# barbararoessle/e2e_multi_view_matching

Measured on AMD Instinct MI355X. Metric: image-pairs/sec @1024 kpts + pose AUC@5/10/20deg vs reference, higher is better.
Workload: dtype f16x2 (fp32 operands carried as 2 fp16 planes hi + 2^-11 lo', 22 significant bits, 3 fp16-MFMA products, fp32 accumulate; same 1e-4 / bit-exact-index parity bar); 1 GPU; configs[1]: tuple_size=2 (1 pair per tuple), 1024 keypoints, 256-dim f32 descriptors, GNN 9x1 = 18 layers, 100 Sinkhorn iters, batch 32 tuples/GPU = 32 pairs/GPU, w8pt pose per pair; pairs_per_gpu=32, global_pairs=32, weights=random init (timed), identity-like for the AUC leg, parallelism=tuple-sharded x1

## Files before the change

e2e_multi_view_matching_amd/csrc/attention_p2w.hip:

```cpp
#include <algorithm>
#include <type_traits>

#include "attention_p2.h"

namespace e2emv {

typedef __attribute__((ext_vector_type(16))) float aw_f32x16;

constexpr int AW_QT = 256;
constexpr int AW_TILEB = 64 * 256;
constexpr int AW_REGB = 2 * AW_TILEB;
constexpr int AW_ELS = 3 * AW_REGB;
constexpr int AW_QIMG = AW_ELS + 2048;
constexpr int AW_LDS = AW_QIMG + 3 * AW_TILEB;
constexpr int AW_PART_F = 68;
constexpr float AW_SINV = 1.f / P2_QS, AW_PLOG = 7.f, AW_LIMIT = 60000.f;

__device__ __forceinline__ void aw_wait_q_k0(p2_f16x8 (&q)[2][2][4]) {
    asm volatile("s_waitcnt vmcnt(0) lgkmcnt(0)\n\ts_barrier"
                 : "+a"(q[0][0][0]), "+a"(q[0][0][1]), "+a"(q[0][0][2]), "+a"(q[0][0][3]), "+a"(q[0][1][0]), "+a"(q[0][1][1]), "+a"(q[0][1][2]), "+a"(q[0][1][3]),
                   "+a"(q[1][0][0]), "+a"(q[1][0][1]), "+a"(q[1][0][2]), "+a"(q[1][0][3]), "+a"(q[1][1][0]), "+a"(q[1][1][1]), "+a"(q[1][1][2]), "+a"(q[1][1][3])
                 :: "memory");
}

template <int I, int N, class F>
__device__ __forceinline__ void aw_for(F&& f) {
    if constexpr (I < N) {
        f(std::integral_constant<int, I>{});
        aw_for<I + 1, N>(f);
    }
}

__device__ __forceinline__ unsigned aw_cvt_pk(float v0, float v1) {
    const p2_f32x2 vv = {v0, v1};
    return __builtin_bit_cast(unsigned, __builtin_convertvector(vv, p2_f16x2));
}
__device__ __forceinline__ float aw_fma(float a, float b, float c) {
    float d;
    asm volatile("v_fma_f32 %0, %1, %2, %3" : "=v"(d) : "v"(a), "v"(b), "v"(c));
    return d;
}
__device__ __forceinline__ float aw_exp2(float a) {
    float d;
    asm volatile("v_exp_f32 %0, %1" : "=v"(d) : "v"(a));
    return d;
}
__device__ __forceinline__ void aw_acc(float& sum, float a) { asm volatile("v_add_f32 %0, %0, %1" : "+v"(sum) : "v"(a)); }
__device__ __forceinline__ unsigned aw_cvt_pk_v(float v0, float v1) {
    unsigned d;
    asm volatile("v_cvt_pk_f16_f32 %0, %1, %2" : "=v"(d) : "v"(v0), "v"(v1));
    return d;
}
__device__ __forceinline__ unsigned aw_mixlo(unsigned hi, float v0) {
    unsigned lo;
    asm volatile("v_fma_mixlo_f16 %0, %1, -1.0, %2 op_sel_hi:[1,0,0]" : "=v"(lo) : "v"(hi), "v"(v0));
    return lo;
}
__device__ __forceinline__ unsigned aw_mixhi(unsigned lo, unsigned hi, float v1) {
    asm volatile("v_fma_mixhi_f16 %0, %1, -1.0, %2 op_sel:[1,0,0] op_sel_hi:[1,0,0]" : "+v"(lo) : "v"(hi), "v"(v1));
    return lo;
}
__device__ __forceinline__ unsigned aw_lo(unsigned hi, float v0, float v1) {
    unsigned lo;
    asm("v_fma_mixlo_f16 %0, %1, -1.0, %2 op_sel_hi:[1,0,0]\n\tv_fma_mixhi_f16 %0, %1, -1.0, %3 op_sel:[1,0,0] op_sel_hi:[1,0,0]"
        : "=&v"(lo) : "v"(hi), "v"(v0), "v"(v1));
    return lo;
}

__device__ __forceinline__ void aw_mfma_s(aw_f32x16& c, p2_f16x8 a, p2_f16x8 b) {
    asm volatile("v_mfma_f32_32x32x16_f16 %0, %1, %2, %0" : "+v"(c) : "v"(a), "a"(b));
}
__device__ __forceinline__ void aw_mfma_s0(aw_f32x16& c, p2_f16x8 a, p2_f16x8 b) {
    asm volatile("v_mfma_f32_32x32x16_f16 %0, %1, %2, 0" : "=&v"(c) : "v"(a), "a"(b));
}
__device__ __forceinline__ void aw_mfma_sa(aw_f32x16& c, p2_f16x8 a, p2_f16x8 b) {
    asm volatile("v_mfma_f32_32x32x16_f16 %0, %1, %2, %0" : "+v"(c) : "a"(a), "a"(b));
}
__device__ __forceinline__ void aw_mfma_sa0(aw_f32x16& c, p2_f16x8 a, p2_f16x8 b) {
    asm volatile("v_mfma_f32_32x32x16_f16 %0, %1, %2, 0" : "=&v"(c) : "a"(a), "a"(b));
}
__device__ __forceinline__ void aw_mfma_oa(aw_f32x16& c, p2_f16x8 a, p2_u32x4 b) {
    asm volatile("v_mfma_f32_32x32x16_f16 %0, %1, %2, %0" : "+a"(c) : "a"(a), "v"(b));
}
template <int IMM>
__device__ __forceinline__ void aw_read_frag(p2_f16x8& d, unsigned addr) {
    static_assert(IMM >= 0 && IMM < 65536, "ds_read offset: 16 bits");
    asm volatile("ds_read_b128 %0, %1 offset:%2" : "=a"(d) : "v"(addr), "n"(IMM));
}
template <int N>
__device__ __forceinline__ void aw_wait_frag(p2_f16x8 (&f)[4]) {
    asm volatile("s_waitcnt lgkmcnt(%4)" : "+a"(f[0]), "+a"(f[1]), "+a"(f[2]), "+a"(f[3]) : "n"(N));
}
template <bool HAS_E, bool MULTI = true, bool PART = false>
__global__ __launch_bounds__(256, 1) void attention_p2w_kernel(AttnP2Params p) {
    extern __shared__ __attribute__((aligned(16))) char smem_aw[];

    int lin = blockIdx.x, ks = 0;
    constexpr bool part = PART;
    if constexpr (PART) {
        const int h = blockIdx.x, tpx = (8 * p.gper * p.nq - p.n_full) >> 3;
        ks = (h >> 3) / tpx;
        lin = p.n_full + 8 * ((h >> 3) % tpx) + (h & 7);
    }
    const int xcd = lin & 7, idx = lin >> 3;
    const int g = xcd * p.gper + idx / p.nq;
    if (g >= p.groups) return;
    const int qt = idx % p.nq;
    const int img = g / p.H, head = g % p.H;
    const int b = img / p.T, t = img % p.T;
    if (qt * AW_QT >= p.nv[t]) return;

    const int tid = threadIdx.x, lane = tid & 63;
    const int wave = __builtin_amdgcn_readfirstlane(tid >> 6);
    const int l31 = lane & 31, lh = lane >> 5;
    const unsigned row_b = 8u * (unsigned)p.D;

    int q_row[2];
    bool q_ok[2];
    p2_f16x8 Qf[2][2][4];
#pragma unroll
    for (int a = 0; a < 2; ++a) {
        q_row[a] = qt * AW_QT + wave * 64 + a * 32 + l31;
        q_ok[a] = q_row[a] < p.n_rows;
    }
    const int q_blk = __builtin_amdgcn_readfirstlane(((int64_t)img * p.n_rows + min(qt * AW_QT + wave * 64, p.n_rows - 1)) >> 6);
    const int e_q_v = HAS_E ? p.EQK[q_blk * 8 + head] : 0;
    const unsigned q_img = wave == 0 ? 2u * AW_REGB : (unsigned)(AW_QIMG + (wave - 1) * AW_TILEB);
    {
        const __amdgpu_buffer_rsrc_t rsQ = __builtin_amdgcn_make_buffer_rsrc(const_cast<uint16_t*>(p.qk), 0, (int)p.qk_bytes, 0x00020000);
        const unsigned so = (unsigned)(img * p.n_rows) * row_b;
        asm volatile("" ::: "memory");
#pragma unroll
        for (int i = 0; i < 16; ++i) {
            const int rl = 4 * i + (lane >> 4);
            const int row = min(qt * AW_QT + wave * 64 + rl, p.n_rows - 1);
            const unsigned c = (unsigned)((lane & 15) ^ (rl & 15));
            p2_glds16(rsQ, smem_aw + q_img + i * 1024, (unsigned)row * row_b + (unsigned)head * 256u + c * 16u, so);
        }
        asm volatile("" ::: "memory");
    }
    const int e_q = __builtin_amdgcn_readfirstlane(e_q_v);

    const int n_src = p.cross ? p.T - 1 : 1;
    auto src_t = [&](int si) __attribute__((always_inline)) { return !p.cross ? t : (si < t ? si : si + 1); };
    int n_tiles = 0;
    for (int si = 0; si < n_src; ++si) n_tiles += (p.nv[src_t(si)] + 63) / 64;
    int t0 = 0;
    if constexpr (PART) {
        t0 = ks * n_tiles / p.n_split;
        n_tiles = (ks + 1) * n_tiles / p.n_split - t0;
        if (n_tiles <= 0) return;
    }
    struct Cur { int si, kt, nv; unsigned kb, vb; int eb; };
    auto cur_src = [&](Cur& c) __attribute__((always_inline)) {
        const int im = b * p.T + src_t(c.si);
        c.kt = 0;
        c.nv = p.nv[src_t(c.si)];
        c.kb = (unsigned)(im * p.n_rows) * row_b;
        c.vb = (unsigned)((im * p.H + head) * 64) * (unsigned)p.n_rows * 4u;
        c.eb = (im * p.n_rows) >> 6;
    };
    auto cur_next = [&](Cur& c) __attribute__((always_inline)) {
        ++c.kt;
        if constexpr (MULTI) {
            if (c.kt * 64 >= c.nv && c.si + 1 < n_src) { ++c.si; cur_src(c); }
        }
    };
    auto cur_init = [&]() __attribute__((always_inline)) {
        Cur c;
        c.si = 0;
        cur_src(c);
        if constexpr (PART)
            for (int i = 0; i < t0; ++i) cur_next(c);
        return c;
    };

    const __amdgpu_buffer_rsrc_t rsK = __builtin_amdgcn_make_buffer_rsrc(const_cast<uint16_t*>(p.qk), 0, (int)p.qk_bytes, 0x00020000);
    const __amdgpu_buffer_rsrc_t rsV = __builtin_amdgcn_make_buffer_rsrc(const_cast<uint16_t*>(p.vt), 0, (int)p.vt_bytes, 0x00020000);
    unsigned k_vo[4], v_vo[4];
#pragma unroll
    for (int i = 0; i < 4; ++i) {
        const int row = 4 * (wave * 4 + i) + (lane >> 4);
        const unsigned c = (unsigned)((lane & 15) ^ (row & 15));
        k_vo[i] = (unsigned)row * row_b + 4u * (unsigned)p.D + (unsigned)head * 256u + c * 16u;
        v_vo[i] = (unsigned)row * (unsigned)p.n_rows * 4u + c * 16u;
    }
    auto k_so = [&](const Cur& c) __attribute__((always_inline)) { return c.kb + (unsigned)c.kt * 64u * row_b; };
    auto v_so = [&](const Cur& c) __attribute__((always_inline)) { return c.vb + (unsigned)c.kt * 256u; };
    auto k_piece = [&](int region, int i, unsigned so) __attribute__((always_inline)) { p2_glds16(rsK, smem_aw + region * AW_REGB + AW_TILEB + (wave * 4 + i) * 1024, k_vo[i], so); };
    auto v_piece = [&](int region, int i, unsigned so) __attribute__((always_inline)) { p2_glds16(rsV, smem_aw + region * AW_REGB + (wave * 4 + i) * 1024, v_vo[i], so); };
    int* const els = reinterpret_cast<int*>(smem_aw + AW_ELS);
    int ek_mine = 0, ev_mine = 0;
    if (HAS_E && tid < n_tiles) {
        int si = 0, kt = PART ? tid + t0 : tid;
        if constexpr (MULTI) {
            for (; si + 1 < n_src; ++si) {
                const int nt = (p.nv[src_t(si)] + 63) / 64;
                if (kt < nt) break;
                kt -= nt;
            }
        }
        const int blk = (((b * p.T + src_t(si)) * p.n_rows) >> 6) + kt;
        ek_mine = p.EQK[blk * 8 + 4 + head];
        if (p.EVt) ev_mine = p.EVt[blk * 4 + head];
    }
    typedef __attribute__((address_space(3))) const p2_u32x2* lds_pair_t;
    const unsigned els0 = (unsigned)(uintptr_t)(__attribute__((address_space(3))) char*)smem_aw + (unsigned)AW_ELS;
    auto read_e = [&](int tl) __attribute__((always_inline)) {
        return *reinterpret_cast<lds_pair_t>((uintptr_t)(els0 + 8u * (unsigned)min(tl, n_tiles - 1)));
    };

    const int kz = l31 & 15;
    const unsigned lds0 = (unsigned)(uintptr_t)(__attribute__((address_space(3))) char*)smem_aw;
    unsigned R[4][2];
#pragma unroll
    for (int s = 0; s < 4; ++s)
#pragma unroll
        for (int pl = 0; pl < 2; ++pl)
            R[s][pl] = lds0 + (unsigned)(l31 * 256 + ((((s >> 1) * 8 + pl * 4 + 2 * (s & 1) + lh) ^ kz) << 4));
    typedef __attribute__((address_space(3))) const p2_f16x8* lds_frag_t;
    auto frag = [&](int s, int pl, int imm) __attribute__((always_inline)) { return *reinterpret_cast<lds_frag_t>((uintptr_t)(R[s][pl] + (unsigned)imm)); };

    constexpr int PA[3] = {1, 0, 0};
    constexpr int PB[3] = {0, 1, 0};

    aw_f32x16 O[2][2], S[2][2];
    p2_u32x4 Pf[2][2][4];
#pragma unroll
    for (int a = 0; a < 2; ++a)
#pragma unroll
        for (int d = 0; d < 2; ++d)
#pragma unroll
            for (int r = 0; r < 16; ++r) O[a][d][r] = 0.f;
    float m_run[2] = {-1e30f, -1e30f}, l_run[2] = {0.f, 0.f};
    int e_o = 0;
    bool o_started = false;
    unsigned n_slow = 0;

    auto sm_slow = [&](auto BB, float sinv, int valid) __attribute__((always_inline)) {
        constexpr int B = decltype(BB)::value;
        asm volatile("s_nop 15" : "+v"(S[B][0]), "+v"(S[B][1]), "+a"(O[B][0]), "+a"(O[B][1]));
        if (valid < 64) {
#pragma unroll
            for (int kb = 0; kb < 2; ++kb)
#pragma unroll
                for (int r = 0; r < 16; ++r)
                    if (kb * 32 + (r & 3) + 8 * (r >> 2) + 4 * lh >= valid) S[B][kb][r] = -INFINITY;
        }
        float mx = S[B][0][0];
#pragma unroll
        for (int kb = 0; kb < 2; ++kb)
#pragma unroll
            for (int r = 0; r < 16; ++r) mx = fmaxf(mx, S[B][kb][r]);
        {
            float x = mx, y = mx;
            asm volatile("s_nop 1\n\tv_permlane32_swap_b32 %0, %1\n\ts_nop 1" : "+v"(x), "+v"(y));
            mx = fmaxf(x, y);
        }
        mx *= sinv;
        const float m_new = fmaxf(m_run[B], mx);
        const float alpha = __builtin_amdgcn_exp2f(m_run[B] - m_new);
#pragma unroll
        for (int r = 0; r < 16; ++r) { O[B][0][r] *= alpha; O[B][1][r] *= alpha; }
        const float e0 = AW_PLOG - m_new;
        float ps = 0.f;
#pragma unroll
        for (int k = 0; k < 16; ++k) {
            const int kb = k >> 3, r = 2 * (k & 7), u = 2 * kb + ((k & 7) >> 2), e = k & 3;
            const float p0 = __builtin_amdgcn_exp2f(__builtin_fmaf(S[B][kb][r], sinv, e0));
            const float p1 = __builtin_amdgcn_exp2f(__builtin_fmaf(S[B][kb][r + 1], sinv, e0));
            ps += p0 + p1;
            const P2Pair pr = p2_split_plain(p0, p1);
            Pf[B][0][u][e] = pr.hi; Pf[B][1][u][e] = pr.lo;
        }
        l_run[B] = l_run[B] * alpha + ps;
        m_run[B] = m_new;
        asm volatile("s_nop 4" : "+a"(O[B][0]), "+a"(O[B][1]));
    };

    Cur cK = cur_init(), cV = cur_init(), cS = cur_init();
    int nK = 0, nV = 0;
    auto adv_k = [&]() __attribute__((always_inline)) { if (++nK < n_tiles) cur_next(cK); };
    auto adv_v = [&]() __attribute__((always_inline)) { if (++nV < n_tiles) cur_next(cV); };
    {
        const unsigned so = k_so(cK);
#pragma unroll
        for (int i = 0; i < 4; ++i) k_piece(2, i, so);
        adv_k();
    }
    unsigned so_v01[2], so_k12[2];
#pragma unroll
    for (int r = 0; r < 2; ++r) {
        so_v01[r] = v_so(cV);
        so_k12[r] = k_so(cK);
        adv_v();
        adv_k();
    }
    if (HAS_E && tid < n_tiles) { els[2 * tid] = ek_mine; els[2 * tid + 1] = ev_mine; }
#pragma unroll
    for (int s = 0; s < 4; ++s)
#pragma unroll
        for (int pl = 0; pl < 2; ++pl) R[s][pl] += q_img;
    asm volatile("s_waitcnt vmcnt(4)" ::: "memory");
    aw_for<0, 16>([&](auto II) __attribute__((always_inline)) {
        constexpr int a = decltype(II)::value >> 3, pl = (decltype(II)::value >> 2) & 1, s = decltype(II)::value & 3;
        aw_read_frag<a * 8192>(Qf[a][pl][s], R[s][pl]);
    });
    aw_wait_q_k0(Qf);
    p2_u32x2 e_pair = {0u, 0u};
    if constexpr (HAS_E) e_pair = read_e(0);
#pragma unroll
    for (int s = 0; s < 4; ++s)
#pragma unroll
        for (int pl = 0; pl < 2; ++pl) R[s][pl] += 2 * AW_REGB - q_img;
    {
        const float sinv = AW_SINV * p2_exp2i(e_q + __builtin_amdgcn_readfirstlane((int)e_pair[0]));
        p2_f16x8 kf[2][2][2];
#pragma unroll
        for (int kb = 0; kb < 2; ++kb)
#pragma unroll
            for (int pl = 0; pl < 2; ++pl) kf[0][kb][pl] = frag(0, pl, AW_TILEB + kb * 8192);
#pragma unroll
        for (int s = 0; s < 4; ++s) {
            if (s < 3) {
#pragma unroll
                for (int kb = 0; kb < 2; ++kb)
#pragma unroll
                    for (int pl = 0; pl < 2; ++pl) kf[(s + 1) & 1][kb][pl] = frag(s + 1, pl, AW_TILEB + kb * 8192);
            }
            __builtin_amdgcn_sched_barrier(0);
#pragma unroll
            for (int a = 0; a < 2; ++a)
#pragma unroll
                for (int q = 0; q < 3; ++q)
#pragma unroll
                    for (int kb = 0; kb < 2; ++kb) {
                        if (s == 0 && q == 0) aw_mfma_s0(S[a][kb], kf[s & 1][kb][PA[q]], Qf[a][PB[q]][s]);
                        else aw_mfma_s(S[a][kb], kf[s & 1][kb][PA[q]], Qf[a][PB[q]][s]);
                        const int slot = s * 12 + a * 6 + q * 2 + kb;
                        if (slot % 3 == 1) {
                            const int n = slot / 3, r = n >> 3, i = n & 3;
                            if ((n & 4) == 0) v_piece(r, i, so_v01[r]);
                            else k_piece(r, i, so_k12[r]);
                        }
                        __builtin_amdgcn_sched_barrier(0);
                    }
        }
        asm volatile("s_waitcnt vmcnt(8) lgkmcnt(0)\n\ts_barrier" ::: "memory");
        sm_slow(std::integral_constant<int, 0>{}, sinv, cS.nv - cS.kt * 64);
        if (cS.nv - cS.kt * 64 >= 64) {
            asm volatile("s_nop 15" : "+v"(S[1][0]), "+v"(S[1][1]));
            float mx = S[1][0][0];
#pragma unroll
            for (int kb = 0; kb < 2; ++kb)
#pragma unroll
                for (int r = 0; r < 16; ++r) mx = fmaxf(mx, S[1][kb][r]);
            float x = mx, y = mx;
            asm volatile("s_nop 1\n\tv_permlane32_swap_b32 %0, %1\n\ts_nop 1" : "+v"(x), "+v"(y));
            m_run[1] = fmaxf(x, y) * sinv;
        }
    }
#pragma unroll
    for (int s = 0; s < 4; ++s)
#pragma unroll
        for (int pl = 0; pl < 2; ++pl) R[s][pl] -= 2 * AW_REGB;
    int reg_cur = 0, seg_tile = 0;

    p2_f16x8 FA[8][4];
    auto read_frag = [&](auto GG, auto NN, auto SS, auto KK) __attribute__((always_inline)) {
        constexpr int G = decltype(GG)::value, N = decltype(NN)::value, S = decltype(SS)::value, KPART = decltype(KK)::value;
        constexpr int x = N & 1, pl = N < 2 ? 1 : 0;
        aw_read_frag<KPART * AW_TILEB + x * 8192>(FA[G][N], R[S][pl]);
    };
    aw_for<0, 8>([&](auto II) __attribute__((always_inline)) {
        constexpr int g = decltype(II)::value / 4, n = decltype(II)::value % 4;
        read_frag(std::integral_constant<int, g>{}, std::integral_constant<int, n>{}, std::integral_constant<int, g>{}, std::integral_constant<int, 0>{});
    });

    auto seg = [&](auto AA, auto LL) __attribute__((always_inline)) {
        constexpr int A = decltype(AA)::value, B = 1 - A;
        constexpr bool LAST = decltype(LL)::value;
        constexpr bool HAS_SM = !(LAST && A == 1);
        constexpr int NSLOT = LAST ? 24 : 48, NG = NSLOT / 6;
        constexpr int MPS = LAST ? 2 : 1;

        if (A == 0) {
            if (HAS_E && p.EVt) {
                const int e_v = __builtin_amdgcn_readfirstlane((int)e_pair[1]);
                if (__builtin_expect(o_started && e_v != e_o, 0)) {
                    const float f = e_o - e_v < -126 ? 0.f : p2_exp2i(e_o - e_v);
                    asm volatile("s_nop 15" : "+a"(O[0][0]), "+a"(O[0][1]), "+a"(O[1][0]), "+a"(O[1][1]));
#pragma unroll
                    for (int a = 0; a < 2; ++a)
#pragma unroll
                        for (int r = 0; r < 16; ++r) { O[a][0][r] *= f; O[a][1][r] *= f; }
                    asm volatile("s_nop 4" : "+a"(O[0][0]), "+a"(O[0][1]), "+a"(O[1][0]), "+a"(O[1][1]));
                }
                e_o = e_v;
                o_started = true;
            }
        }
        float sinv = AW_SINV, e0 = 0.f, ps = 0.f;
        int valid = 64;
        if (HAS_SM) {
            if (HAS_E) sinv = AW_SINV * p2_exp2i(e_q + __builtin_amdgcn_readfirstlane((int)e_pair[0]));
            if (HAS_E && A == 0 && !LAST) e_pair = read_e(seg_tile + 1);
            e0 = AW_PLOG - m_run[B];
            valid = cS.nv - cS.kt * 64;
        }
        if (HAS_SM && __builtin_expect(valid < 64, 0)) {
            asm volatile("s_nop 7" : "+v"(S[B][0]), "+v"(S[B][1]));
#pragma unroll
            for (int kb = 0; kb < 2; ++kb)
#pragma unroll
                for (int r = 0; r < 16; ++r)
                    if (kb * 32 + (r & 3) + 8 * (r >> 2) + 4 * lh >= valid) S[B][kb][r] = -INFINITY;
            asm volatile("" : "+v"(S[B][0]), "+v"(S[B][1]));
        }
        bool slow = false;
        float xa[16][2], pa[16][2], psA = 0.f, psB = 0.f, sinv_v = sinv;
        asm volatile("" : "+v"(sinv_v), "+v"(e0));
        unsigned hi_k[16], lo_k[16];
        auto micro = [&](auto MM) __attribute__((always_inline)) {
            constexpr int m = decltype(MM)::value;
            constexpr int k = m / 3, ph = m % 3;
            constexpr int kb = (k & 15) >> 3, r = 2 * (k & 7);
            if constexpr (m == 48) {
                lo_k[15] = aw_mixlo(hi_k[15], pa[15][0]);
            } else if constexpr (m == 49) {
                Pf[B][1][3][3] = aw_mixhi(lo_k[15], hi_k[15], pa[15][1]);
            } else if constexpr (ph == 0) {
                xa[k][0] = aw_fma(S[B][kb][r], sinv_v, e0);
                if constexpr (k > 0) lo_k[k - 1] = aw_mixlo(hi_k[k - 1], pa[k - 1][0]);
                xa[k][1] = aw_fma(S[B][kb][r + 1], sinv_v, e0);
            } else if constexpr (ph == 1) {
                pa[k][0] = aw_exp2(xa[k][0]);
                if constexpr (k > 0) {
                    constexpr int k1 = k - 1, u = 2 * (k1 >> 3) + ((k1 & 7) >> 2), e = k1 & 3;
                    Pf[B][1][u][e] = aw_mixhi(lo_k[k1], hi_k[k1], pa[k1][1]);
                }
                pa[k][1] = aw_exp2(xa[k][1]);
            } else {
                constexpr int u = 2 * (k >> 3) + ((k & 7) >> 2), e = k & 3;
                aw_acc(psA, pa[k][0]);
                hi_k[k] = aw_cvt_pk_v(pa[k][0], pa[k][1]);
                Pf[B][0][u][e] = hi_k[k];
                aw_acc(psB, pa[k][1]);
            }
        };

        unsigned so_v = 0, so_k = 0;
        if (A == 0 && !LAST) {
            so_v = v_so(cV);
            adv_v();
            so_k = k_so(cK);
            adv_k();
        }
        const int reg_ld = reg_cur == 0 ? 2 : reg_cur - 1;

        aw_for<0, NSLOT>([&](auto II) __attribute__((always_inline)) {
            constexpr int i = decltype(II)::value;
            constexpr int gq = i / 6, w = i % 6;
            if constexpr (A == 0 && w == 0) aw_wait_frag<(gq + 1 < NG ? 4 : 0)>(FA[gq]);
            if constexpr (i < 24) {
                constexpr int u = i / 6, q = (i % 6) / 2, db = i % 2;
                aw_mfma_oa(O[A][db], FA[u][db + 2 * (1 - PA[q])], Pf[A][PB[q]][u]);
            } else {
                constexpr int s = (i - 24) / 6, q = (i % 6) / 2, kb = i % 2;
                if constexpr (s == 0 && q == 0) aw_mfma_sa0(S[A][kb], FA[4 + s][kb + 2 * (1 - PA[q])], Qf[A][PB[q]][s]);
                else aw_mfma_sa(S[A][kb], FA[4 + s][kb + 2 * (1 - PA[q])], Qf[A][PB[q]][s]);
            }
            if constexpr (HAS_SM) {
                if constexpr (LAST) {
                    aw_for<0, MPS>([&](auto JJ) __attribute__((always_inline)) { micro(std::integral_constant<int, MPS * i + decltype(JJ)::value>{}); });
                } else if constexpr (i < 9) {
                    constexpr int m0 = i + i / 2 - (i > 0 && i % 2 == 0 ? 1 : 0);
                    micro(std::integral_constant<int, m0>{});
                    if constexpr (i >= 2 && i % 2 == 0) micro(std::integral_constant<int, m0 + 1>{});
                } else if constexpr (i < 46) {
                    micro(std::integral_constant<int, i + 4>{});
                } else if constexpr (i == 46) {
                    ps = psA;
                    aw_acc(ps, psB);
                } else if constexpr (i == 47) {
                    slow = __builtin_amdgcn_ballot_w64(!(ps < AW_LIMIT)) != 0;
                    l_run[B] += slow ? 0.f : ps;
                }
            }
            if constexpr (A == 1 && !LAST && i == 36) {
                asm volatile("s_waitcnt vmcnt(8) lgkmcnt(0)\n\ts_barrier" ::: "memory");
                const unsigned d = reg_cur == 2 ? (unsigned)(-2 * AW_REGB) : (unsigned)AW_REGB;
#pragma unroll
                for (int s = 0; s < 4; ++s)
#pragma unroll
                    for (int pl = 0; pl < 2; ++pl) R[s][pl] += d;
                reg_cur = reg_cur == 2 ? 0 : reg_cur + 1;
            }
            if constexpr (w >= 1 && w <= 4) {
                constexpr int gn = gq + 2;
                constexpr auto N = std::integral_constant<int, w - 1>{};
                if constexpr (A == 0 && gn < NG) {
                    if constexpr (gn < 4) read_frag(std::integral_constant<int, gn>{}, N, std::integral_constant<int, gn>{}, std::integral_constant<int, 0>{});
                    else read_frag(std::integral_constant<int, gn>{}, N, std::integral_constant<int, gn - 4>{}, std::integral_constant<int, 1>{});
                } else if constexpr (A == 1 && !LAST && gn >= NG) {
                    read_frag(std::integral_constant<int, gn - NG>{}, N, std::integral_constant<int, gn - NG>{}, std::integral_constant<int, 0>{});
                }
            }
            if constexpr (A == 0 && !LAST && i < 32 && i % 4 == 1) {
                if constexpr (i < 16) v_piece(reg_ld, i / 4, so_v);
                else k_piece(reg_ld, i / 4 - 4, so_k);
            }
            __builtin_amdgcn_sched_barrier(0);
        });

        if constexpr (HAS_SM && LAST) {
            lo_k[15] = aw_mixlo(hi_k[15], pa[15][0]);
            ps = psA + psB;
            Pf[B][1][3][3] = aw_mixhi(lo_k[15], hi_k[15], pa[15][1]);
            const bool slow = __builtin_amdgcn_ballot_w64(!(ps < AW_LIMIT)) != 0;
            l_run[B] += slow ? 0.f : ps;
            if (__builtin_expect(slow, 0)) {
                sm_slow(std::integral_constant<int, B>{}, sinv, valid);
                ++n_slow;
            }
        }
        if constexpr (HAS_SM && !LAST) {
            if (__builtin_expect(slow, 0)) {
                sm_slow(std::integral_constant<int, B>{}, sinv, valid);
                ++n_slow;
            }
        }
        if (A == 0) cur_next(cS);
    };

    for (int j = 0; j + 1 < n_tiles; ++j) {
        seg_tile = j;
        seg(std::integral_constant<int, 0>{}, std::false_type{});
        seg(std::integral_constant<int, 1>{}, std::false_type{});
    }
    seg(std::integral_constant<int, 0>{}, std::true_type{});
    seg(std::integral_constant<int, 1>{}, std::true_type{});

    asm volatile("s_waitcnt vmcnt(0)" ::: "memory");
    asm volatile("s_nop 15" : "+a"(O[0][0]), "+a"(O[0][1]), "+a"(O[1][0]), "+a"(O[1][1]));
    if constexpr (PART) {
        const int64_t rec = ((int64_t)(lin - p.n_full) * p.n_split + ks) * AW_QT;
        if (lane == 0) p.part_e[rec / 64 + wave] = e_o;
#pragma unroll
        for (int a = 0; a < 2; ++a) {
            const float l_tot = l_run[a] + __shfl_xor(l_run[a], 32);
            float* o = p.part + (rec + wave * 64 + a * 32 + l31) * AW_PART_F;
#pragma unroll
            for (int d = 0; d < 2; ++d)
#pragma unroll
                for (int gq = 0; gq < 4; ++gq)
                    *reinterpret_cast<p2_f32x4*>(o + 32 * d + 8 * gq + 4 * lh) = p2_f32x4{O[a][d][4 * gq], O[a][d][4 * gq + 1], O[a][d][4 * gq + 2], O[a][d][4 * gq + 3]};
            if (lh == 0) { o[64] = m_run[a]; o[65] = l_tot; }
        }
        if (p.stats && n_slow && lane == 0) atomicAdd(p.stats, n_slow);
        return;
    }
    if (p.EO && lane == 0 && q_ok[0]) p.EO[(((int64_t)img * p.n_rows + q_row[0]) >> 6) * 4 + head] = e_o;
#pragma unroll
    for (int a = 0; a < 2; ++a) {
        const float l_tot = l_run[a] + __shfl_xor(l_run[a], 32);
        const float inv = 1.f / (l_tot * P2_VS);
        uint16_t* op = p.out + p2_index((int64_t)img * p.n_rows + q_row[a], head * 64, p.D) + 8 * lh;
#pragma unroll
        for (int d = 0; d < 2; ++d)
#pragma unroll
            for (int kp = 0; kp < 2; ++kp) {
                const int r0 = 8 * kp, r1 = 8 * kp + 4;
                const P2Pair x0 = p2_split_scaled(O[a][d][r0] * inv, O[a][d][r0 + 1] * inv), x1 = p2_split_scaled(O[a][d][r0 + 2] * inv, O[a][d][r0 + 3] * inv);
                const P2Pair y0 = p2_split_scaled(O[a][d][r1] * inv, O[a][d][r1 + 1] * inv), y1 = p2_split_scaled(O[a][d][r1 + 2] * inv, O[a][d][r1 + 3] * inv);
                const auto h0 = __builtin_amdgcn_permlane32_swap(x0.hi, y0.hi, false, false), h1 = __builtin_amdgcn_permlane32_swap(x1.hi, y1.hi, false, false);
                const auto l0 = __builtin_amdgcn_permlane32_swap(x0.lo, y0.lo, false, false), l1 = __builtin_amdgcn_permlane32_swap(x1.lo, y1.lo, false, false);
                uint16_t* o = op + d * 64 + kp * 16;
                if (q_ok[a]) {
                    *reinterpret_cast<p2_u32x4*>(o) = p2_u32x4{h0[0], h1[0], h0[1], h1[1]};
                    *reinterpret_cast<p2_u32x4*>(o + 32) = p2_u32x4{l0[0], l1[0], l0[1], l1[1]};
                }
            }
    }
    if (p.stats && n_slow && lane == 0) atomicAdd(p.stats, n_slow);
}

__global__ __launch_bounds__(1024) void attention_p2w_combine(AttnP2Params p) {
    const int item = blockIdx.x, lin = p.n_full + item;
    const int xcd = lin & 7, idx = lin >> 3;
    const int g = xcd * p.gper + idx / p.nq;
    if (g >= p.groups) return;
    const int qt = idx % p.nq, img = g / p.H, head = g % p.H, t = img % p.T;
    if (qt * AW_QT >= p.nv[t]) return;
    const int n_src = p.cross ? p.T - 1 : 1;
    int n_tiles = 0;
    for (int si = 0; si < n_src; ++si) n_tiles += (p.nv[!p.cross ? t : (si < t ? si : si + 1)] + 63) / 64;
    const int q = threadIdx.x >> 2, dq = (threadIdx.x & 3) * 16;
    const int row = qt * AW_QT + q;
    float m = -3.0e38f;
    int e = -1000;
    for (int k = 0; k < p.n_split; ++k) {
        if ((k + 1) * n_tiles / p.n_split - k * n_tiles / p.n_split <= 0) continue;
        const int64_t rec = ((int64_t)item * p.n_split + k) * AW_QT;
        m = fmaxf(m, p.part[(rec + q) * AW_PART_F + 64]);
        e = max(e, p.part_e[rec / 64 + (q >> 6)]);
    }
    float acc[16], l = 0.f;
#pragma unroll
    for (int i = 0; i < 16; ++i) acc[i] = 0.f;
    for (int k = 0; k < p.n_split; ++k) {
        if ((k + 1) * n_tiles / p.n_split - k * n_tiles / p.n_split <= 0) continue;
        const int64_t rec = ((int64_t)item * p.n_split + k) * AW_QT;
        const float* o = p.part + (rec + q) * AW_PART_F;
        const int ek = p.part_e[rec / 64 + (q >> 6)];
        const float a = __builtin_amdgcn_exp2f(o[64] - m);
        const float ae = a * (ek - e < -126 ? 0.f : p2_exp2i(ek - e));
        l += a * o[65];
#pragma unroll
        for (int i = 0; i < 16; i += 4) {
            const p2_f32x4 v = *reinterpret_cast<const p2_f32x4*>(o + dq + i);
            acc[i] += ae * v[0]; acc[i + 1] += ae * v[1]; acc[i + 2] += ae * v[2]; acc[i + 3] += ae * v[3];
        }
    }
    if (row >= p.n_rows) return;
    if (p.EO && (threadIdx.x & 255) == 0) p.EO[(((int64_t)img * p.n_rows + row) >> 6) * 4 + head] = e;
    const float inv = 1.f / (l * P2_VS);
    uint16_t* op = p.out + p2_index((int64_t)img * p.n_rows + row, head * 64 + dq, p.D);
#pragma unroll
    for (int h = 0; h < 2; ++h) {
        p2_u32x4 hi, lo;
#pragma unroll
        for (int i = 0; i < 4; ++i) {
            const P2Pair pr = p2_split_scaled(acc[8 * h + 2 * i] * inv, acc[8 * h + 2 * i + 1] * inv);
            hi[i] = pr.hi; lo[i] = pr.lo;
        }
        *reinterpret_cast<p2_u32x4*>(op + 8 * h) = hi;
        *reinterpret_cast<p2_u32x4*>(op + 8 * h + 32) = lo;
    }
}

int launch_attention_p2w(e2emv_ctx* ctx, AttnP2Params& p, int n_valid, hipStream_t s) {
    p.nq = (n_valid + AW_QT - 1) / AW_QT;
    if (int rc = ensure_flags(ctx)) return rc;
    p.stats = ctx->d_flags + 5;
    const size_t lds = AW_LDS;
    const bool multi = p.cross && p.T > 2;
    const void* fn = p.EQK ? (multi ? reinterpret_cast<const void*>(attention_p2w_kernel<true, true>) : reinterpret_cast<const void*>(attention_p2w_kernel<true, false>))
                           : (multi ? reinterpret_cast<const void*>(attention_p2w_kernel<false, true>) : reinterpret_cast<const void*>(attention_p2w_kernel<false, false>));
    if (int rc = ensure_dynamic_lds(ctx, fn, lds)) return rc;
    void* args[] = {&p};
    const int n_items = 8 * p.gper * p.nq, cus = std::max(8, ctx->num_cus / 8 * 8);
    const int r = n_items % cus;
    const int min_tiles = attn_min_tiles(p, 64);
    p.n_full = n_items;
    p.n_split = 1;
    p.part = nullptr;
    p.part_e = nullptr;
    if (ctx->attn_key_split && r > 0 && 2 * r <= cus && r % 8 == 0) {
        const int k = std::min(std::min(cus / r, 8), min_tiles);
        if (k >= 2) {
            const size_t n_rec = (size_t)r * k * AW_QT;
            const size_t need = n_rec * AW_PART_F * sizeof(float) + (n_rec / 64) * sizeof(int);
            if (need > ctx->attn_part_bytes) {
                if (ctx->d_attn_part) { E2EMV_HIP(ctx, hipStreamSynchronize(s)); (void)hipFree(ctx->d_attn_part); ctx->d_attn_part = nullptr; ctx->attn_part_bytes = 0; }
                E2EMV_HIP(ctx, hipMalloc((void**)&ctx->d_attn_part, need));
                ctx->attn_part_bytes = need;
            }
            p.n_full = n_items - r;
            p.n_split = k;
            p.part = ctx->d_attn_part;
            p.part_e = reinterpret_cast<int*>(ctx->d_attn_part + n_rec * AW_PART_F);
        }
    }
    if (p.n_full > 0) {
        E2EMV_HIP(ctx, hipLaunchKernel(fn, dim3(p.n_full), dim3(256), args, lds, s));
        E2EMV_CHECK_LAUNCH(ctx, "attention_p2w_kernel");
    }
    if (p.n_split > 1) {
        const void* fp = p.EQK ? (multi ? reinterpret_cast<const void*>(attention_p2w_kernel<true, true, true>) : reinterpret_cast<const void*>(attention_p2w_kernel<true, false, true>))
                               : (multi ? reinterpret_cast<const void*>(attention_p2w_kernel<false, true, true>) : reinterpret_cast<const void*>(attention_p2w_kernel<false, false, true>));
        if (int rc = ensure_dynamic_lds(ctx, fp, lds)) return rc;
        E2EMV_HIP(ctx, hipLaunchKernel(fp, dim3((n_items - p.n_full) * p.n_split), dim3(256), args, lds, s));
        E2EMV_CHECK_LAUNCH(ctx, "attention_p2w_kernel (parts)");
        hipLaunchKernelGGL(attention_p2w_combine, dim3(n_items - p.n_full), dim3(1024), 0, s, p);
        E2EMV_CHECK_LAUNCH(ctx, "attention_p2w_combine");
    }
    return E2EMV_OK;
}

}
```

Before: 3534 pairs/s.

## Overlap first-tile softmax of block 0 with block 1 QK MFMAs in prologue

The prologue of the attention kernel is reordered. It computes the block-0 score MFMAs first, then interleaves block 0's exp/split/pack softmax micro-steps with block 1's score MFMAs, instead of running all MFMAs and then a serial sm_slow pass. K fragments for all four slices are now prefetched into a 4-deep register buffer. The per-tile softmax micro-op lambda is factored into a shared sm_micro with a variant that sums the row in a different order. The cost is higher register pressure, and the changed summation order may shift low-order bits of the row sums.

```diff
diff --git a/e2e_multi_view_matching_amd/csrc/attention_p2w.hip b/e2e_multi_view_matching_amd/csrc/attention_p2w.hip
--- a/e2e_multi_view_matching_amd/csrc/attention_p2w.hip
+++ b/e2e_multi_view_matching_amd/csrc/attention_p2w.hip
@@ -46,6 +46,11 @@
     return d;
 }
 __device__ __forceinline__ void aw_acc(float& sum, float a) { asm volatile("v_add_f32 %0, %0, %1" : "+v"(sum) : "v"(a)); }
+__device__ __forceinline__ float aw_add(float a, float b) {
+    float d;
+    asm volatile("v_add_f32 %0, %1, %2" : "=v"(d) : "v"(a), "v"(b));
+    return d;
+}
 __device__ __forceinline__ unsigned aw_cvt_pk_v(float v0, float v1) {
     unsigned d;
     asm volatile("v_cvt_pk_f16_f32 %0, %1, %2" : "=v"(d) : "v"(v0), "v"(v1));
@@ -278,6 +283,39 @@
         asm volatile("s_nop 4" : "+a"(O[B][0]), "+a"(O[B][1]));
     };
 
+    struct SmState { float xa[16][2], pa[16][2], t[16], psA, psB, sinv, e0; unsigned hi[16], lo[16]; };
+    auto sm_micro = [&](auto BB, auto ONE, auto MM, SmState& z) __attribute__((always_inline)) {
+        constexpr int B = decltype(BB)::value, m = decltype(MM)::value;
+        constexpr bool one = decltype(ONE)::value;
+        constexpr int k = m / 3, ph = m % 3;
+        constexpr int kb = (k & 15) >> 3, r = 2 * (k & 7);
+        if constexpr (m == 48) {
+            z.lo[15] = aw_mixlo(z.hi[15], z.pa[15][0]);
+        } else if constexpr (m == 49) {
+            Pf[B][1][3][3] = aw_mixhi(z.lo[15], z.hi[15], z.pa[15][1]);
+        } else if constexpr (ph == 0) {
+            z.xa[k][0] = aw_fma(S[B][kb][r], z.sinv, z.e0);
+            if constexpr (k > 0) z.lo[k - 1] = aw_mixlo(z.hi[k - 1], z.pa[k - 1][0]);
+            z.xa[k][1] = aw_fma(S[B][kb][r + 1], z.sinv, z.e0);
+        } else if constexpr (ph == 1) {
+            z.pa[k][0] = aw_exp2(z.xa[k][0]);
+            if constexpr (k > 0) {
+                constexpr int k1 = k - 1, u = 2 * (k1 >> 3) + ((k1 & 7) >> 2), e = k1 & 3;
+                Pf[B][1][u][e] = aw_mixhi(z.lo[k1], z.hi[k1], z.pa[k1][1]);
+            }
+            z.pa[k][1] = aw_exp2(z.xa[k][1]);
+        } else {
+            constexpr int u = 2 * (k >> 3) + ((k & 7) >> 2), e = k & 3;
+            if constexpr (one && k > 0) aw_acc(z.psA, z.t[k - 1]);
+            else aw_acc(z.psA, z.pa[k][0]);
+            z.hi[k] = aw_cvt_pk_v(z.pa[k][0], z.pa[k][1]);
+            Pf[B][0][u][e] = z.hi[k];
+            if constexpr (one && k > 0) z.t[k] = aw_add(z.pa[k][0], z.pa[k][1]);
+            else if constexpr (one) z.t[k] = z.pa[k][1];
+            else aw_acc(z.psB, z.pa[k][1]);
+        }
+    };
+
     Cur cK = cur_init(), cV = cur_init(), cS = cur_init();
     int nK = 0, nV = 0;
     auto adv_k = [&]() __attribute__((always_inline)) { if (++nK < n_tiles) cur_next(cK); };
@@ -301,6 +339,7 @@
     for (int s = 0; s < 4; ++s)
 #pragma unroll
         for (int pl = 0; pl < 2; ++pl) R[s][pl] += q_img;
+    asm volatile("" : "+a"(O[0][0]), "+a"(O[0][1]), "+a"(O[1][0]), "+a"(O[1][1]));
     asm volatile("s_waitcnt vmcnt(4)" ::: "memory");
     aw_for<0, 16>([&](auto II) __attribute__((always_inline)) {
         constexpr int a = decltype(II)::value >> 3, pl = (decltype(II)::value >> 2) & 1, s = decltype(II)::value & 3;
@@ -315,40 +354,74 @@
         for (int pl = 0; pl < 2; ++pl) R[s][pl] += 2 * AW_REGB - q_img;
     {
         const float sinv = AW_SINV * p2_exp2i(e_q + __builtin_amdgcn_readfirstlane((int)e_pair[0]));
-        p2_f16x8 kf[2][2][2];
+        const int valid0 = cS.nv - cS.kt * 64;
+        p2_f16x8 kf[4][2][2];
+        auto read_k0 = [&](int s) __attribute__((always_inline)) {
+#pragma unroll
+            for (int kb = 0; kb < 2; ++kb)
+#pragma unroll
+                for (int pl = 0; pl < 2; ++pl) kf[s][kb][pl] = frag(s, pl, AW_TILEB + kb * 8192);
+        };
+        auto late_piece = [&](int slot) __attribute__((always_inline)) {
+            if (slot % 3 == 1) {
+                const int n = slot / 3, r = n >> 3, i = n & 3;
+                if ((n & 4) == 0) v_piece(r, i, so_v01[r]);
+                else k_piece(r, i, so_k12[r]);
+            }
+        };
+        read_k0(0);
+        read_k0(1);
+#pragma unroll
+        for (int s = 0; s < 4; ++s) {
+            if (s < 2) read_k0(s + 2);
+            __builtin_amdgcn_sched_barrier(0);
+#pragma unroll
+            for (int q = 0; q < 3; ++q)
+#pragma unroll
+                for (int kb = 0; kb < 2; ++kb) {
+                    if (s == 0 && q == 0) aw_mfma_s0(S[0][kb], kf[s][kb][PA[q]], Qf[0][PB[q]][s]);
+                    else aw_mfma_s(S[0][kb], kf[s][kb][PA[q]], Qf[0][PB[q]][s]);
+                    late_piece(s * 6 + q * 2 + kb);
+                    __builtin_amdgcn_sched_barrier(0);
+                }
+        }
+        asm volatile("s_nop 15" : "+v"(S[0][0]), "+v"(S[0][1]));
+        if (__builtin_expect(valid0 < 64, 0)) {
+#pragma unroll
+            for (int kb = 0; kb < 2; ++kb)
+#pragma unroll
+                for (int r = 0; r < 16; ++r)
+                    if (kb * 32 + (r & 3) + 8 * (r >> 2) + 4 * lh >= valid0) S[0][kb][r] = -INFINITY;
+            asm volatile("" : "+v"(S[0][0]), "+v"(S[0][1]));
+        }
+        float m0 = S[0][0][0];
 #pragma unroll
         for (int kb = 0; kb < 2; ++kb)
 #pragma unroll
-            for (int pl = 0; pl < 2; ++pl) kf[0][kb][pl] = frag(0, pl, AW_TILEB + kb * 8192);
-#pragma unroll
-        for (int s = 0; s < 4; ++s) {
-            if (s < 3) {
-#pragma unroll
-                for (int kb = 0; kb < 2; ++kb)
-#pragma unroll
-                    for (int pl = 0; pl < 2; ++pl) kf[(s + 1) & 1][kb][pl] = frag(s + 1, pl, AW_TILEB + kb * 8192);
-            }
+            for (int r = 0; r < 16; ++r) m0 = fmaxf(m0, S[0][kb][r]);
+        {
+            float x = m0, y = m0;
+            asm volatile("s_nop 1\n\tv_permlane32_swap_b32 %0, %1\n\ts_nop 1" : "+v"(x), "+v"(y));
+            m0 = fmaxf(m_run[0], fmaxf(x, y) * sinv);
+        }
+        SmState z;
+        z.psA = 0.f; z.sinv = sinv; z.e0 = AW_PLOG - m0;
+        asm volatile("" : "+v"(z.sinv), "+v"(z.e0));
+        aw_for<0, 24>([&](auto II) __attribute__((always_inline)) {
+            constexpr int i = decltype(II)::value;
+            constexpr int s = i / 6, q = (i % 6) / 2, kb = i % 2;
+            if constexpr (s == 0 && q == 0) aw_mfma_s0(S[1][kb], kf[s][kb][PA[q]], Qf[1][PB[q]][s]);
+            else aw_mfma_s(S[1][kb], kf[s][kb][PA[q]], Qf[1][PB[q]][s]);
+            constexpr int m_lo = i < 22 ? 2 * i : 44 + 3 * (i - 22), m_hi = i < 22 ? m_lo + 2 : m_lo + 3;
+            aw_for<m_lo, m_hi>([&](auto MM) __attribute__((always_inline)) { sm_micro(std::integral_constant<int, 0>{}, std::true_type{}, MM, z); });
+            late_piece(24 + i);
             __builtin_amdgcn_sched_barrier(0);
-#pragma unroll
-            for (int a = 0; a < 2; ++a)
-#pragma unroll
-                for (int q = 0; q < 3; ++q)
-#pragma unroll
-                    for (int kb = 0; kb < 2; ++kb) {
-                        if (s == 0 && q == 0) aw_mfma_s0(S[a][kb], kf[s & 1][kb][PA[q]], Qf[a][PB[q]][s]);
-                        else aw_mfma_s(S[a][kb], kf[s & 1][kb][PA[q]], Qf[a][PB[q]][s]);
-                        const int slot = s * 12 + a * 6 + q * 2 + kb;
-                        if (slot % 3 == 1) {
-                            const int n = slot / 3, r = n >> 3, i = n & 3;
-                            if ((n & 4) == 0) v_piece(r, i, so_v01[r]);
-                            else k_piece(r, i, so_k12[r]);
-                        }
-                        __builtin_amdgcn_sched_barrier(0);
-                    }
-        }
+        });
+        aw_acc(z.psA, z.t[15]);
+        l_run[0] = z.psA;
+        m_run[0] = m0;
         asm volatile("s_waitcnt vmcnt(8) lgkmcnt(0)\n\ts_barrier" ::: "memory");
-        sm_slow(std::integral_constant<int, 0>{}, sinv, cS.nv - cS.kt * 64);
-        if (cS.nv - cS.kt * 64 >= 64) {
+        if (valid0 >= 64) {
             asm volatile("s_nop 15" : "+v"(S[1][0]), "+v"(S[1][1]));
             float mx = S[1][0][0];
 #pragma unroll
@@ -400,7 +473,7 @@
                 o_started = true;
             }
         }
-        float sinv = AW_SINV, e0 = 0.f, ps = 0.f;
+        float sinv = AW_SINV, e0 = 0.f;
         int valid = 64;
         if (HAS_SM) {
             if (HAS_E) sinv = AW_SINV * p2_exp2i(e_q + __builtin_amdgcn_readfirstlane((int)e_pair[0]));
@@ -418,36 +491,11 @@
             asm volatile("" : "+v"(S[B][0]), "+v"(S[B][1]));
         }
         bool slow = false;
-        float xa[16][2], pa[16][2], psA = 0.f, psB = 0.f, sinv_v = sinv;
-        asm volatile("" : "+v"(sinv_v), "+v"(e0));
-        unsigned hi_k[16], lo_k[16];
-        auto micro = [&](auto MM) __attribute__((always_inline)) {
-            constexpr int m = decltype(MM)::value;
-            constexpr int k = m / 3, ph = m % 3;
-            constexpr int kb = (k & 15) >> 3, r = 2 * (k & 7);
-            if constexpr (m == 48) {
-                lo_k[15] = aw_mixlo(hi_k[15], pa[15][0]);
-            } else if constexpr (m == 49) {
-                Pf[B][1][3][3] = aw_mixhi(lo_k[15], hi_k[15], pa[15][1]);
-            } else if constexpr (ph == 0) {
-                xa[k][0] = aw_fma(S[B][kb][r], sinv_v, e0);
-                if constexpr (k > 0) lo_k[k - 1] = aw_mixlo(hi_k[k - 1], pa[k - 1][0]);
-                xa[k][1] = aw_fma(S[B][kb][r + 1], sinv_v, e0);
-            } else if constexpr (ph == 1) {
-                pa[k][0] = aw_exp2(xa[k][0]);
-                if constexpr (k > 0) {
-                    constexpr int k1 = k - 1, u = 2 * (k1 >> 3) + ((k1 & 7) >> 2), e = k1 & 3;
-                    Pf[B][1][u][e] = aw_mixhi(lo_k[k1], hi_k[k1], pa[k1][1]);
-                }
-                pa[k][1] = aw_exp2(xa[k][1]);
-            } else {
-                constexpr int u = 2 * (k >> 3) + ((k & 7) >> 2), e = k & 3;
-                aw_acc(psA, pa[k][0]);
-                hi_k[k] = aw_cvt_pk_v(pa[k][0], pa[k][1]);
-                Pf[B][0][u][e] = hi_k[k];
-                aw_acc(psB, pa[k][1]);
-            }
-        };
+        float ps = 0.f;
+        SmState z;
+        z.psA = 0.f; z.psB = 0.f; z.sinv = sinv; z.e0 = e0;
+        asm volatile("" : "+v"(z.sinv), "+v"(z.e0));
+        auto micro = [&](auto MM) __attribute__((always_inline)) { sm_micro(std::integral_constant<int, B>{}, std::false_type{}, MM, z); };
 
         unsigned so_v = 0, so_k = 0;
         if (A == 0 && !LAST) {
@@ -480,8 +528,8 @@
                 } else if constexpr (i < 46) {
                     micro(std::integral_constant<int, i + 4>{});
                 } else if constexpr (i == 46) {
-                    ps = psA;
-                    aw_acc(ps, psB);
+                    ps = z.psA;
+                    aw_acc(ps, z.psB);
                 } else if constexpr (i == 47) {
                     slow = __builtin_amdgcn_ballot_w64(!(ps < AW_LIMIT)) != 0;
                     l_run[B] += slow ? 0.f : ps;
@@ -514,9 +562,9 @@
         });
 
         if constexpr (HAS_SM && LAST) {
-            lo_k[15] = aw_mixlo(hi_k[15], pa[15][0]);
-            ps = psA + psB;
-            Pf[B][1][3][3] = aw_mixhi(lo_k[15], hi_k[15], pa[15][1]);
+            z.lo[15] = aw_mixlo(z.hi[15], z.pa[15][0]);
+            ps = z.psA + z.psB;
+            Pf[B][1][3][3] = aw_mixhi(z.lo[15], z.hi[15], z.pa[15][1]);
             const bool slow = __builtin_amdgcn_ballot_w64(!(ps < AW_LIMIT)) != 0;
             l_run[B] += slow ? 0.f : ps;
             if (__builtin_expect(slow, 0)) {
```

New measurement: 3544 pairs/s, median of 5. About the same (+0.3%).
